# feifeibear/long-context-attention

Measured on AMD Instinct MI355X. Metric: attention TFLOP/s (algorithmic, causal fwd+bwd) + iter ms of LongContextAttention at seqlen 64K, ulysses x ring, higher is better.
Workload: dtype bf16

## Files before the change

long-context-attention_amd/csrc/usp_flash_fwd64.hip:

```cpp
#ifdef USP_F64_TIMING
#define USP_TIMING
#endif
#include "usp_fwd_params.hpp"
#include "usp_host.hpp"
#include "usp_mfma64.hpp"

namespace usp {

#ifndef USP_F64_NEA
#define USP_F64_NEA 42
#endif
constexpr int kF64_NEA = USP_F64_NEA;
#ifndef USP_F64_LEAD
#define USP_F64_LEAD 2
#endif
constexpr int kF64_LEAD = USP_F64_LEAD;
#ifndef USP_F64_PFK
#define USP_F64_PFK 2
#endif
constexpr int kF64_PFK = USP_F64_PFK;
#ifndef USP_F64_PFV
#define USP_F64_PFV 2
#endif
constexpr int kF64_PFV = USP_F64_PFV;
#ifndef USP_F64_MAX0
#define USP_F64_MAX0 22
#endif
constexpr int kF64_MAX0 = USP_F64_MAX0;
#ifndef USP_F64_DMA0
#define USP_F64_DMA0 2
#endif
constexpr int kF64_DMA0 = USP_F64_DMA0;
#ifndef USP_F64_DMAS
#define USP_F64_DMAS 6
#endif
constexpr int kF64_DMAS = USP_F64_DMAS;


template <int DT, bool CAUSAL, bool SPLIT = false>
__global__ __launch_bounds__(256, 1) void flash_fwd64_kernel(const FwdArgsT<SPLIT> ) {
  using E = Elem<DT>;
  using M = M64<DT>;
  constexpr int D = 128;
  constexpr int kBM = 256;
  constexpr int ROWB = D * 2;
  constexpr int KBYTES = kBN * ROWB;
  constexpr int NKT = D / 16;
  constexpr int NDJ = D / 32;
  constexpr int VOFF = 2 * KBYTES;

  extern __shared__ __attribute__((aligned(16))) char smem_raw[];
  USP_LDS char* smem = (USP_LDS char*)smem_raw;

  const int tid = threadIdx.x;
  const int lane = tid & 63;
  const int wave = __builtin_amdgcn_readfirstlane(tid >> 6);
  const int l31 = lane & 31;
  const int hi = lane >> 5;
  typedef const __attribute__((address_space(4))) FwdArgsT<SPLIT>* KArgs;
  KArgs p = (KArgs)__builtin_amdgcn_kernarg_segment_ptr();
  asm volatile("" : "+s"(p));

  const int k_voff = (16 * wave + (lane >> 4)) * (int)p->k_ss * 2 + (((lane & 15) ^ (lane >> 4)) * 16);
  const int v_voff = (16 * wave + ((lane & 15) >> 2)) * (int)p->v_ss * 2 + (32 * (lane >> 4) + 8 * (lane & 3)) * 2;
  const int k_rd = l31 * ROWB + ((hi ^ (l31 & 15)) * 16);
  const int v_rd = VOFF + hi * NDJ * 256 + ((lane & 15) >> 2) * 64 + ((lane >> 4) & 1) * 32 + (lane & 3) * 8;
  const float c = p->scale_log2;

  const ItemWalk walk(p->n_items);
  for (int pass = 0;; ++pass) {
  int w = walk.at(pass);
  if (w < 0) break;
  asm volatile("" : "+s"(p));
  int ks = 0;
  if constexpr (SPLIT) {
    w = walk.dealt(w, p->nq * p->ksplit);
    ks = w % p->ksplit; w /= p->ksplit;
  } else {
    w = walk.grouped(walk.dealt(w, p->nq), p->nq, p->walk_g);
  }
  const int qt_r = w % p->nq;
  int rest = w / p->nq;
  const int qt = CAUSAL ? (p->nq - 1 - qt_r) : qt_r;
  const int g = rest % p->G;
  rest /= p->G;
  const int hkv = rest % p->Hkv;
  const int b = rest / p->Hkv;
  const int h = hkv * p->G + g;

  const int q0 = qt * kBM;
  const int qw = q0 + wave * 64;
  int off = p->causal_off;
  int kb = 0, sk_cut = 0;
  if constexpr (SPLIT) {
    int e = p->Sk;
    if (CAUSAL) e = usp_rows_key_end(q0, kBM, p->Sq, e, 1, off);
    const int nt_all = usp_tiles_holding(e, kBN);
    kb = usp_prop_cut_tile(nt_all, p->ksplit, ks) * kBN;
    int ke = (ks == p->ksplit - 1) ? p->Sk : usp_prop_cut_tile(nt_all, p->ksplit, ks + 1) * kBN;
    ke = ke < p->Sk ? ke : p->Sk;
    sk_cut = ke > kb ? ke - kb : 0;
    off -= kb;
  }
  auto n_keys = [&]() { if constexpr (SPLIT) return sk_cut; else return p->Sk; };

  int blk_kv_end = n_keys(), wave_kv_end = n_keys();
  if (CAUSAL) {
    const int blk_last = (q0 + kBM < p->Sq ? q0 + kBM : p->Sq) - 1;
    const int wav_last = (qw + 64 < p->Sq ? qw + 64 : p->Sq) - 1;
    blk_kv_end = blk_last + off + 1 < n_keys() ? blk_last + off + 1 : n_keys();
    wave_kv_end = wav_last + off + 1 < n_keys() ? wav_last + off + 1 : n_keys();
  }
  if (qw >= p->Sq) wave_kv_end = 0;
  const int nt = usp_tiles_holding(blk_kv_end, kBN);
  int n_full = usp_unmasked_tiles(qw, n_keys(), CAUSAL, off, kBN);
  if (n_full > nt) n_full = nt;

USP_TM(
  const uint64_t tm_item = __builtin_amdgcn_s_memtime();
)
  u32x4 qf[2][NKT];
#pragma unroll
  for (int qb = 0; qb < 2; ++qb) {
    const int row = qw + 32 * qb + l31;
    const int row_c = row < p->Sq ? row : p->Sq - 1;
    const char* qp = p->q + 2 * (b * p->q_sb + (int64_t)row_c * p->q_ss + h * p->q_sh) + 16 * hi;
#pragma unroll
    for (int t = 0; t < NKT; ++t) qf[qb][t] = *(const u32x4*)(qp + 32 * t);
  }
#pragma unroll
  for (int qb = 0; qb < 2; ++qb)
#pragma unroll
    for (int t = 0; t < NKT; ++t) pin_agpr4(qf[qb][t]);

  const int64_t k_tb = (int64_t)kBN * p->k_ss * 2, v_tb = (int64_t)kBN * p->v_ss * 2;
  const char* k_cur = p->k + 2 * (b * p->k_sb + hkv * p->k_sh);
  const char* v_cur = p->v + 2 * (b * p->v_sb + hkv * p->v_sh);
  if constexpr (SPLIT) { k_cur += 2 * (int64_t)kb * p->k_ss; v_cur += 2 * (int64_t)kb * p->v_ss; }
  int rows_kv = n_keys();
  const int k_rowb = (int)p->k_ss * 2, v_rowb = (int)p->v_ss * 2;
  int lds_w = wave * 4096, k_step = 4 * (int)p->k_ss * 2 - 1024, v_step = 4 * (int)p->v_ss * 2 - 1024;
  u32x4 k_rs, v_rs;
  int k_ahead = 0;
  int dma_kbuf = 0, dma_vbuf = 0;
  auto dma_open = [&](int kbuf, int vbuf) {
    k_rs = make_rsrc_rows(k_cur, rows_kv + kBN * k_ahead, kBN, k_rowb, 2 * D);
    v_rs = make_rsrc_rows(v_cur, rows_kv, kBN, v_rowb, 2 * D);
    k_cur += k_tb;
    v_cur += v_tb;
    rows_kv -= kBN;
    dma_kbuf = kbuf; dma_vbuf = vbuf;
  };
  auto dma_open_k = [&](int kbuf) {
    k_rs = make_rsrc_rows(k_cur, rows_kv, kBN, k_rowb, 2 * D);
    k_cur += k_tb;
    k_ahead = -1;
    dma_kbuf = kbuf;
  };
  auto dma_piece = [&](int n) {
    asm volatile("" : "+s"(lds_w), "+s"(k_step), "+s"(v_step));
    if (n < 4) lds_dma16_asm(k_rs, lds_w + dma_kbuf * KBYTES, k_voff ^ (64 * n), n * k_step, n);
    else lds_dma16_asm(v_rs, lds_w + VOFF + dma_vbuf * KBYTES, v_voff, (n - 4) * v_step, n - 4);
  };
  auto dma_all = [&](int kbuf, int vbuf) {
    dma_open(kbuf, vbuf);
#pragma unroll
    for (int n = 0; n < 8; ++n) dma_piece(n);
  };

  f32x16 o[2][NDJ];
#pragma unroll
  for (int qb = 0; qb < 2; ++qb)
#pragma unroll
    for (int dj = 0; dj < NDJ; ++dj) zero_pin_agpr(o[qb][dj]);
  float m_run[2] = {USP_NEG_INF, USP_NEG_INF};
  float l_run[2] = {0.f, 0.f};

  auto qk = [&](int kbuf, f32x16 (&s)[2][2]) {
#pragma unroll
    for (int kt = 0; kt < NKT; ++kt) {
      USP_LDS const char* kp = smem + kbuf * KBYTES + (k_rd ^ (32 * kt));
      const u32x4 k0 = *(USP_LDS const u32x4*)kp;
      const u32x4 k1 = *(USP_LDS const u32x4*)(kp + 32 * ROWB);
#pragma unroll
      for (int qb = 0; qb < 2; ++qb) {
        if (kt == 0) { M::template s_first<true>(s[qb][0], k0, qf[qb][0]); M::template s_first<true>(s[qb][1], k1, qf[qb][0]); }
        else { M::template s_next<true>(s[qb][0], k0, qf[qb][kt]); M::template s_next<true>(s[qb][1], k1, qf[qb][kt]); }
      }
    }
    mfma_settle(s);
  };
  auto mask = [&](int kt0, f32x16 (&s)[2][2]) {
#pragma unroll
    for (int qb = 0; qb < 2; ++qb) {
      const int row = qw + 32 * qb + l31;
      int klim = n_keys() - 1;
      if (CAUSAL) klim = row + off < klim ? row + off : klim;
      const int kb0 = kt0 + 4 * hi;
#pragma unroll
      for (int r = 0; r < 16; ++r) {
        const int key = kb0 + (r & 3) + 8 * (r >> 2);
        if (key > klim) s[qb][0][r] = USP_NEG_INF;
        if (key + 32 > klim) s[qb][1][r] = USP_NEG_INF;
      }
    }
  };
  f32x16 sa[2][2], sb[2][2];
#pragma unroll
  for (int qb = 0; qb < 2; ++qb)
#pragma unroll
    for (int kb = 0; kb < 2; ++kb)
#pragma unroll
      for (int r = 0; r < 16; ++r) { sa[qb][kb][r] = 0.f; sb[qb][kb][r] = 0.f; }
  dma_all(0, 0);
  dma_open_k(1);
#pragma unroll
  for (int n = 0; n < 4; ++n) dma_piece(n);
  dma_drain();
  __syncthreads();
  if (nt > 0 && wave_kv_end > 0) qk(0, sa);
  __syncthreads();

  constexpr float kThr = 8.f;
  constexpr int NA = 32, NB = 32;
  constexpr int NEA = kF64_NEA, LEAD = kF64_LEAD, PFK = kF64_PFK, PFV = kF64_PFV, MAX0 = kF64_MAX0;
  constexpr int DMA0 = kF64_DMA0, DMAS = kF64_DMAS;
  static_assert(64 - NEA <= 22, "k-step 3 of P must be complete two slots before slot 24 of phase B");
  static_assert(MAX0 >= 1 && MAX0 < NB && DMAS >= 1 && DMA0 + 7 * DMAS < NA + NB, "");
  const float thr_raw = kThr / c;
  float m_thr[2] = {USP_NEG_INF, USP_NEG_INF};
  float nmc[2] = {0.f, 0.f};
  auto first_ref = [&](const float (&mt_lane)[2]) {
#pragma unroll
    for (int qb = 0; qb < 2; ++qb) {
      const float m_new = xhalf_max(mt_lane[qb]);
      const float m_use = (m_new == USP_NEG_INF) ? 0.f : m_new;
      m_run[qb] = m_new;
      m_thr[qb] = m_new + thr_raw;
      nmc[qb] = -(m_use * c);
    }
  };
  auto rescale = [&](const float (&mt_lane)[2]) {
    asm volatile("; rescale (rare)" ::: "memory");
    mfma_settle(o);
#pragma unroll
    for (int qb = 0; qb < 2; ++qb) {
      const float m_new = fmaxf(m_run[qb], xhalf_max(mt_lane[qb]));
      const float m_use = (m_new == USP_NEG_INF) ? 0.f : m_new;
      const float alpha = (m_new == m_run[qb]) ? 1.f : fast_exp2(m_run[qb] * c - m_use * c);
      m_run[qb] = m_new;
      m_thr[qb] = m_new + thr_raw;
      nmc[qb] = -(m_use * c);
      l_run[qb] *= alpha;
#pragma unroll
      for (int dj = 0; dj < NDJ; ++dj)
#pragma unroll
        for (int r = 0; r < 16; ++r) o[qb][dj][r] *= alpha;
    }
#pragma unroll
    for (int qb = 0; qb < 2; ++qb)
#pragma unroll
      for (int dj = 0; dj < NDJ; ++dj) pin_agpr(o[qb][dj]);
    operand_settle();
  };
  auto decide = [&](f32x16 (&s)[2][2]) {
    float mt[2];
#pragma unroll
    for (int qb = 0; qb < 2; ++qb) {
      mt[qb] = s[qb][0][0];
#pragma unroll
      for (int r = 1; r < 16; ++r) mt[qb] = fmaxf(mt[qb], s[qb][0][r]);
#pragma unroll
      for (int r = 0; r < 16; ++r) mt[qb] = fmaxf(mt[qb], s[qb][1][r]);
    }
    first_ref(mt);
  };
  auto iter = [&](auto par_c, auto mode_c, int jpar, int kt0_next, f32x16 (&cs)[2][2], f32x16 (&ns)[2][2])
      __attribute__((always_inline)) {
    constexpr int PARV = decltype(par_c)::value, MODE = decltype(mode_c)::value;
    const int par = PARV < 2 ? PARV : jpar;
    dma_open(par, par ^ 1);
    auto dma_slot = [&](int g) {
      if (g >= DMA0 && (g - DMA0) % DMAS == 0 && (g - DMA0) / DMAS < 8) dma_piece((g - DMA0) / DMAS);
    };
    USP_LDS const char* kb = smem + (par ^ 1) * KBYTES;
    USP_LDS const char* vb = smem + par * KBYTES + v_rd;
    int kr = k_rd;
    asm volatile("" : "+v"(kr));
    u32x4 ka[2 * NKT];
    auto rd_k = [&](int f) {
      ka[f] = *(USP_LDS const u32x4*)(kb + (f & 1) * 32 * ROWB + (kr ^ (32 * (f >> 1))));
    };
    u32x4 va[4 * NDJ];
    auto rd_v = [&](int f) {
      USP_LDS const char* vp = vb + (4 * (f / NDJ) * NDJ + (f % NDJ)) * 256;
      const u32x2 v0 = lds_read_tr16(vp);
      const u32x2 v1 = lds_read_tr16(vp + 2 * NDJ * 256);
      va[f] = u32x4{v0[0], v0[1], v1[0], v1[1]};
    };
    float rs[2] = {0.f, 0.f};
    u32x4 pf[2][4];
    auto get = [&](int e) -> float { return cs[(e >> 3) & 1][e >> 5][8 * ((e >> 4) & 1) + (e & 7)]; };
    auto consume = [&](int e) {
      rs[(e >> 3) & 1] += get(e);
      if (e & 1) pf[(e >> 3) & 1][e >> 4][(e & 7) >> 1] = E::pack2(get(e - 1), get(e));
    };
    auto exp_elem = [&](int e) {
      cs[(e >> 3) & 1][e >> 5][8 * ((e >> 4) & 1) + (e & 7)] = fast_exp2(__builtin_fmaf(get(e), c, nmc[(e >> 3) & 1]));
      if (e > 0) consume(e - 1);
      if (e == 63) consume(63);
    };
    if (MODE != 2) {
#pragma unroll
      for (int f = 0; f < PFK; ++f) rd_k(f);
    }
#pragma unroll
    for (int e = 0; e < LEAD; ++e) exp_elem(e);
    __builtin_amdgcn_sched_barrier(0);
#pragma unroll
    for (int sl = 0; sl < NA; ++sl) {
      const int f = sl >> 1, kt = f >> 1, kbk = f & 1, qb = sl & 1;
      if (MODE != 2) {
        if (qb == 0 && f + PFK < 2 * NKT) rd_k(f + PFK);
        if (kt == 0) M::template s_first<MODE != 0>(ns[qb][kbk], ka[f], qf[qb][0]);
        else M::template s_next<MODE != 0>(ns[qb][kbk], ka[f], qf[qb][kt]);
      }
#pragma unroll
      for (int e = LEAD + sl * (NEA - LEAD) / NA; e < LEAD + (sl + 1) * (NEA - LEAD) / NA; ++e) exp_elem(e);
      if (sl >= NA - 2 * PFV && ((sl - (NA - 2 * PFV)) & 1) == 0) rd_v((sl - (NA - 2 * PFV)) >> 1);
      dma_slot(sl);
      __builtin_amdgcn_sched_barrier(0);
    }
    if (MODE == 1) {
      mfma_settle(ns);
      mask(kt0_next, ns);
    }
    float mt[2] = {USP_NEG_INF, USP_NEG_INF};
    bool keep = true;
    constexpr int NMAX = NB - MAX0;
#pragma unroll
    for (int i = 0; i < NB; ++i) {
      const int f = i >> 1, qb = i & 1;
      if (qb == 0 && f + PFV < 4 * NDJ) rd_v(f + PFV);
      M::template o_acc<MODE != 0>(o[qb][f % NDJ], va[f], pf[qb][f / NDJ]);
      if (NEA + i < 64) exp_elem(NEA + i);
      if (i == 64 - NEA - 1 || (NEA == 64 && i == 0)) { l_run[0] += rs[0]; l_run[1] += rs[1]; }
      if (MODE != 2 && i >= MAX0) {
#pragma unroll
        for (int x = (i - MAX0) * 64 / NMAX; x < (i - MAX0 + 1) * 64 / NMAX; ++x)
          mt[x >> 5] = fmaxf(mt[x >> 5], ns[x >> 5][(x >> 4) & 1][x & 15]);
        if (i == NB - 1) keep = __all(mt[0] <= m_thr[0] && mt[1] <= m_thr[1]);
      }
      dma_slot(NA + i);
      __builtin_amdgcn_sched_barrier(0);
    }
    if (!keep) rescale(mt);
    dma_drain();
    __syncthreads();
  };

  const int n_w = usp_tiles_holding(wave_kv_end, kBN);
  if (n_full > n_w) n_full = n_w;
  int j = 0;
USP_TM(
  const uint64_t tm_loop = __builtin_amdgcn_s_memtime();
  uint64_t tm_hot = tm_loop;
)
  if (n_w > 0) {
    if (n_full == 0) mask(0, sa);
    decide(sa);
    const std::integral_constant<int, 0> c0;
    const std::integral_constant<int, 1> c1;
    const std::integral_constant<int, 2> c2;
    const int n_hot = n_full - 1;
    for (; j + 1 < n_hot; j += 2) {
      iter(c0, c0, 0, 0, sa, sb);
      iter(c1, c0, 1, 0, sb, sa);
    }
    auto adopt = [&]() {
#pragma unroll
      for (int qb = 0; qb < 2; ++qb)
#pragma unroll
        for (int kb = 0; kb < 2; ++kb) sa[qb][kb] = sb[qb][kb];
    };
USP_TM(
    tm_hot = __builtin_amdgcn_s_memtime();
)
    if (j < n_hot) { iter(c0, c0, 0, 0, sa, sb); adopt(); ++j; }
    for (; j < n_w; ++j) {
      if (j + 1 >= n_w) iter(c2, c2, j & 1, 0, sa, sb);
      else { iter(c2, c1, j & 1, (j + 1) * kBN, sa, sb); adopt(); }
    }
  }
USP_TM(
  const uint64_t tm_own = __builtin_amdgcn_s_memtime();
)
  for (; j < nt; ++j) {
    dma_all(j & 1, (j + 1) & 1);
    dma_drain();
    __syncthreads();
  }

USP_TM(
  const uint64_t tm_idle = __builtin_amdgcn_s_memtime();
)
  mfma_settle(o);
  asm volatile("" : "+s"(p));
#pragma unroll
  for (int qb = 0; qb < 2; ++qb) {
    const int row = qw + 32 * qb + l31;
    const float l_tot = xhalf_sum(l_run[qb]);
    const bool empty = !(l_tot > 0.f);
    const float inv = empty ? 0.f : 1.f / l_tot;
    const float blk_lse = empty ? USP_NEG_INF : (m_run[qb] * c + log2f(l_tot)) * kLn2;
    float w_blk = inv, w_old = 0.f, new_lse = blk_lse;
    float* lse_p = p->lse + b * p->lse_sb + h * p->lse_sh + row;
    if constexpr (SPLIT) lse_p += (int64_t)ks * p->B * p->Hq * p->Sq;
    const bool valid = row < p->Sq;
    const bool fin = row >= p->final_begin && row < p->final_end;
    const bool wide = !p->merge_in && p->out_wide && __all(!valid || fin);
    if (valid) {
      if (p->merge_in) {
        const float old = *lse_p;
        const float mx = fmaxf(old, blk_lse);
        if (mx == USP_NEG_INF) {
          new_lse = USP_NEG_INF; w_old = 0.f; w_blk = 0.f;
        } else {
          const float e_old = exp2f((old - mx) * kLog2e);
          const float e_blk = exp2f((blk_lse - mx) * kLog2e);
          const float sum = e_old + e_blk;
          new_lse = mx + log2f(sum) * kLn2;
          w_old = e_old / sum;
          w_blk = e_blk / sum * inv;
        }
      }
      if (hi == 0) *lse_p = new_lse;
      int64_t arow = b * p->a_sb + (int64_t)row * p->a_ss + h * p->a_sh;
      if constexpr (SPLIT) arow += (int64_t)ks * p->B * p->Sq * p->Hq * D;
      const int64_t orow = b * p->o_sb + (int64_t)row * p->o_ss + h * p->o_sh;
      if (wide) {
        char* op = p->out + 2 * orow;
#pragma unroll
        for (int dj = 0; dj < NDJ; ++dj)
#pragma unroll
          for (int g2 = 0; g2 < 2; ++g2) {
            const int r0 = 8 * g2;
            uint32_t ax = E::pack2(o[qb][dj][r0] * w_blk, o[qb][dj][r0 + 1] * w_blk);
            uint32_t ay = E::pack2(o[qb][dj][r0 + 2] * w_blk, o[qb][dj][r0 + 3] * w_blk);
            uint32_t bx = E::pack2(o[qb][dj][r0 + 4] * w_blk, o[qb][dj][r0 + 5] * w_blk);
            uint32_t by = E::pack2(o[qb][dj][r0 + 6] * w_blk, o[qb][dj][r0 + 7] * w_blk);
            const auto sx = __builtin_amdgcn_permlane32_swap(ax, bx, false, false);
            const auto sy = __builtin_amdgcn_permlane32_swap(ay, by, false, false);
            *(u32x4*)(op + 2 * (32 * dj + 16 * g2 + 8 * hi)) = u32x4{sx[0], sy[0], sx[1], sy[1]};
          }
      } else {
#pragma unroll
        for (int dj = 0; dj < NDJ; ++dj) {
#pragma unroll
          for (int g4 = 0; g4 < 4; ++g4) {
            const int d0 = 32 * dj + 8 * g4 + 4 * hi;
            f32x4 val = {o[qb][dj][4 * g4] * w_blk, o[qb][dj][4 * g4 + 1] * w_blk, o[qb][dj][4 * g4 + 2] * w_blk,
                         o[qb][dj][4 * g4 + 3] * w_blk};
            if (p->merge_in) {
              const f32x4 a = *(const f32x4*)(p->acc + arow + d0);
              val += a * w_old;
            }
            if (fin) {
              u32x2 pk = {E::pack2(val[0], val[1]), E::pack2(val[2], val[3])};
              *(u32x2*)(p->out + 2 * (orow + d0)) = pk;
            } else {
              *(f32x4*)(p->acc + arow + d0) = val;
            }
          }
        }
      }
    }
  }
USP_TM(
  {
    const uint64_t tm_end = __builtin_amdgcn_s_memtime();
    if (lane == 0 && (blockIdx.x % 61) == 0 && pass < 4)
      printf("TF wg %3d pass %d wave %d qt %2d tiles own %3d wg %3d : prologue %6llu hot-loop %8llu (%5llu / tile) tail-tiles %6llu idle %6llu epilogue %6llu\n",
             (int)blockIdx.x, pass, wave, qt, n_w, nt, (unsigned long long)(tm_loop - tm_item), (unsigned long long)(tm_hot - tm_loop),
             (unsigned long long)((tm_hot - tm_loop) / (n_full > 2 ? (n_full - 1) / 2 * 2 : 1)), (unsigned long long)(tm_own - tm_hot),
             (unsigned long long)(tm_idle - tm_own), (unsigned long long)(tm_end - tm_idle));
  }
)
  }
}

template <bool SPLIT>
static int launch64(FwdArgsT<SPLIT>& p, int dtype, bool causal, hipStream_t st) {
  p.nq = (p.Sq + 255) / 256;
  p.n_items = p.B * p.Hq * p.nq;
  if constexpr (SPLIT) p.n_items *= p.ksplit;
  const int grid = persistent_grid(p.n_items, device_cus(), p.interleave);
  const size_t lds = 2 * 2 * kBN * 128 * 2;
  with_dtype_causal(dtype, causal, [&](auto dt, auto c) {
    hipLaunchKernelGGL((flash_fwd64_kernel<decltype(dt)::value, decltype(c)::value, SPLIT>), dim3(grid), dim3(256), lds, st, p);
  });
  return launched();
}

bool launch_fwd64(const FwdArgsT<true>& p_in, int dtype, bool causal, hipStream_t st, int* rc) {
  if (!dma_rows_ok(p_in.k_ss, true) || !dma_rows_ok(p_in.v_ss, false)) return false;
  if (p_in.win_on || p_in.seq_q) return false;
  if (p_in.ksplit > 1) {
    FwdArgsT<true> p = p_in;
    p.acc = p.ws_o;
    p.a_sb = (int64_t)p.Sq * p.Hq * 128; p.a_ss = (int64_t)p.Hq * 128; p.a_sh = 128;
    p.lse = p.ws_lse;
    p.lse_sb = (int64_t)p.Hq * p.Sq; p.lse_sh = p.Sq;
    p.merge_in = 0; p.final_begin = 0; p.final_end = 0; p.out_wide = 0;
    *rc = launch64(p, dtype, causal, st);
    if (*rc == USP_OK) *rc = launch_split_merge(p_in, dtype, 128, st);
  } else {
    FwdArgsT<false> p;
    static_cast<FwdParams&>(p) = p_in;
    *rc = launch64(p, dtype, causal, st);
  }
  return true;
}

}
```

long-context-attention_amd/csrc/usp_mfma64.hpp:

```cpp
#pragma once
#include "usp_common.hpp"

#ifdef USP_TIMING
#define USP_TM(...) __VA_ARGS__
#else
#define USP_TM(...)
#endif

namespace usp {

USP_DEV USP_LDS char* lds_block_at_zero(char* smem_raw) {
  if ((uint32_t)(uintptr_t)(USP_LDS char*)smem_raw != 0u) __builtin_trap();
  return (USP_LDS char*)(uintptr_t)0;
}

template <int DT> struct M64;
#if defined(__HIP_DEVICE_COMPILE__)
#define USP_M64_BODY(MN)                                                                                              \
              \
   \
   \
  template <bool SAFE = false> static USP_DEV void s_first(f32x16& s, const u32x4& a, const u32x4& q) {               \
    if (SAFE) asm volatile("s_nop 1\n\t" MN " %0, %1, %2, 0" : "=&v"(s) : "v"(a), "a"(q));                          \
    else asm volatile(MN " %0, %1, %2, 0" : "=&v"(s) : "v"(a), "a"(q));                                               \
  }                                                                                                                   \
            \
  template <bool SAFE = false> static USP_DEV void s_first_c(f32x16& s, const u32x4& a, const u32x4& q, const f32x16& c) { \
    if (SAFE) asm volatile("s_nop 1\n\t" MN " %0, %1, %2, %3" : "=&v"(s) : "v"(a), "a"(q), "v"(c));                \
    else asm volatile(MN " %0, %1, %2, %3" : "=&v"(s) : "v"(a), "a"(q), "v"(c));                                      \
  }                                                                                                                   \
  template <bool SAFE = false> static USP_DEV void s_next(f32x16& s, const u32x4& a, const u32x4& q) {                \
    if (SAFE) asm volatile("s_nop 1\n\t" MN " %0, %1, %2, %0" : "+v"(s) : "v"(a), "a"(q));                          \
    else asm volatile(MN " %0, %1, %2, %0" : "+v"(s) : "v"(a), "a"(q));                                               \
  }                                                                                                                   \
                                             \
  template <bool SAFE = false> static USP_DEV void o_acc(f32x16& o, const u32x4& a, const u32x4& b) {                 \
    if (SAFE) asm volatile("s_nop 1\n\t" MN " %0, %1, %2, %0" : "+a"(o) : "v"(a), "v"(b));                          \
    else asm volatile(MN " %0, %1, %2, %0" : "+a"(o) : "v"(a), "v"(b));                                               \
  }
#else
#define USP_M64_BODY(MN)                                                                                              \
  template <bool SAFE = false> static USP_DEV void s_first(f32x16&, const u32x4&, const u32x4&) {}                    \
  template <bool SAFE = false> static USP_DEV void s_first_c(f32x16&, const u32x4&, const u32x4&, const f32x16&) {}   \
  template <bool SAFE = false> static USP_DEV void s_next(f32x16&, const u32x4&, const u32x4&) {}                     \
  template <bool SAFE = false> static USP_DEV void o_acc(f32x16&, const u32x4&, const u32x4&) {}
#endif
template <> struct M64<0> { USP_M64_BODY("v_mfma_f32_32x32x16_bf16") };
template <> struct M64<1> { USP_M64_BODY("v_mfma_f32_32x32x16_f16") };

USP_DEV void pin_agpr4(u32x4& x) {
#if defined(__HIP_DEVICE_COMPILE__)
  asm volatile("" : "+a"(x));
#endif
}
USP_DEV void zero_pin_agpr(f32x16& o) {
#pragma unroll
  for (int r = 0; r < 16; ++r) o[r] = 0.f;
  pin_agpr(o);
}
USP_DEV void load_resident16(u32x4 (&f0)[8], u32x4 (&f1)[8], const char* r0, const char* r1) {
#if defined(__HIP_DEVICE_COMPILE__)
  asm volatile("global_load_dwordx4 %0, %16, off\n\tglobal_load_dwordx4 %1, %16, off offset:32\n\t"
               "global_load_dwordx4 %2, %16, off offset:64\n\tglobal_load_dwordx4 %3, %16, off offset:96\n\t"
               "global_load_dwordx4 %4, %16, off offset:128\n\tglobal_load_dwordx4 %5, %16, off offset:160\n\t"
               "global_load_dwordx4 %6, %16, off offset:192\n\tglobal_load_dwordx4 %7, %16, off offset:224\n\t"
               "global_load_dwordx4 %8, %17, off\n\tglobal_load_dwordx4 %9, %17, off offset:32\n\t"
               "global_load_dwordx4 %10, %17, off offset:64\n\tglobal_load_dwordx4 %11, %17, off offset:96\n\t"
               "global_load_dwordx4 %12, %17, off offset:128\n\tglobal_load_dwordx4 %13, %17, off offset:160\n\t"
               "global_load_dwordx4 %14, %17, off offset:192\n\tglobal_load_dwordx4 %15, %17, off offset:224\n\t"
               "s_waitcnt vmcnt(0)"
               : "=&a"(f0[0]), "=&a"(f0[1]), "=&a"(f0[2]), "=&a"(f0[3]), "=&a"(f0[4]), "=&a"(f0[5]), "=&a"(f0[6]), "=&a"(f0[7]),
                 "=&a"(f1[0]), "=&a"(f1[1]), "=&a"(f1[2]), "=&a"(f1[3]), "=&a"(f1[4]), "=&a"(f1[5]), "=&a"(f1[6]), "=&a"(f1[7])
               : "v"(r0), "v"(r1) : "memory");
#endif
}
USP_DEV void mfma_settle(f32x16 (&o)[2][4]) {
#if defined(__HIP_DEVICE_COMPILE__)
  asm volatile("s_nop 15" : "+a"(o[0][0]), "+a"(o[0][1]), "+a"(o[0][2]), "+a"(o[0][3]),
                            "+a"(o[1][0]), "+a"(o[1][1]), "+a"(o[1][2]), "+a"(o[1][3]));
#endif
}
USP_DEV void mfma_settle(f32x16 (&s)[2][2]) {
  asm volatile("s_nop 15" : "+v"(s[0][0]), "+v"(s[0][1]), "+v"(s[1][0]), "+v"(s[1][1]));
}
USP_DEV void mfma_settle(f32x16 (&s)[2]) { asm volatile("s_nop 15" : "+v"(s[0]), "+v"(s[1])); }
USP_DEV void operand_settle() { asm volatile("s_nop 3" ::: "memory"); }

USP_DEV int dma_lane_col(int l15, int row) { return (l15 ^ (row << 2)) * 16; }
template <int D> USP_DEV int tile_swz(int row);
template <int D> USP_DEV int tr_read_offset(int i, int grp, int hi, int dj, int e) {
  const int rr = 8 * e + 4 * hi + (i >> 2);
  const int slot = 4 * dj + 2 * grp + ((i & 3) >> 1);
  return rr * (D * 2) + ((slot ^ tile_swz<D>(rr)) * 16) + (i & 1) * 8;
}

USP_DEV void lds_dma16_asm(const u32x4& rsrc, int lds_dst, int voffset, int soffset, int piece) {
#if defined(__HIP_DEVICE_COMPILE__)
  if (piece == 0)
    asm volatile("s_mov_b32 m0, %0\n\ts_nop 0\n\tbuffer_load_dwordx4 %1, %2, %3 offen lds"
                 : : "s"(lds_dst), "v"(voffset), "s"(rsrc), "s"(soffset) : "memory");
  if (piece == 1) asm volatile("buffer_load_dwordx4 %0, %1, %2 offen offset:1024 lds" : : "v"(voffset), "s"(rsrc), "s"(soffset) : "memory");
  if (piece == 2) asm volatile("buffer_load_dwordx4 %0, %1, %2 offen offset:2048 lds" : : "v"(voffset), "s"(rsrc), "s"(soffset) : "memory");
  if (piece == 3) asm volatile("buffer_load_dwordx4 %0, %1, %2 offen offset:3072 lds" : : "v"(voffset), "s"(rsrc), "s"(soffset) : "memory");
#endif
}
USP_DEV void lds_dma4_asm(const u32x4& rsrc, int lds_dst, int voffset) {
#if defined(__HIP_DEVICE_COMPILE__)
  asm volatile("s_mov_b32 m0, %0\n\ts_nop 0\n\tbuffer_load_dword %1, %2, 0 offen lds"
               : : "s"(lds_dst), "v"(voffset), "s"(rsrc) : "memory");
#endif
}
USP_DEV u32x4 make_rsrc(const char* base, int64_t bytes) {
  const uint64_t a = (uint64_t)base;
  const uint32_t n = bytes <= 0 ? 0u : (bytes > 0xffffffffLL ? 0xffffffffu : (uint32_t)bytes);
  return u32x4{(uint32_t)a, (uint32_t)(a >> 32) & 0xffffu, n, 0x00020000u};
}

USP_DEV u32x4 make_rsrc_rows(const char* base, int rows, int tile_rows, int row_bytes, int used) {
  const uint64_t a = (uint64_t)base;
  const int r = rows < tile_rows ? rows : tile_rows;
  const int n = r * row_bytes - (row_bytes - used);
  return u32x4{(uint32_t)a, (uint32_t)(a >> 32) & 0xffffu, (uint32_t)(n > 0 ? n : 0), 0x00020000u};
}

template <class E, int NDJ>
USP_DEV void store_row16_wide(char* row, const f32x16 (&t)[NDJ], float mul, int hi, bool valid) {
#if defined(__HIP_DEVICE_COMPILE__)
#pragma unroll
  for (int dj = 0; dj < NDJ; ++dj)
#pragma unroll
    for (int g2 = 0; g2 < 2; ++g2) {
      const int r0 = 8 * g2;
      const uint32_t ax = E::pack2(t[dj][r0] * mul, t[dj][r0 + 1] * mul);
      const uint32_t ay = E::pack2(t[dj][r0 + 2] * mul, t[dj][r0 + 3] * mul);
      const uint32_t bx = E::pack2(t[dj][r0 + 4] * mul, t[dj][r0 + 5] * mul);
      const uint32_t by = E::pack2(t[dj][r0 + 6] * mul, t[dj][r0 + 7] * mul);
      const auto sx = __builtin_amdgcn_permlane32_swap(ax, bx, false, false);
      const auto sy = __builtin_amdgcn_permlane32_swap(ay, by, false, false);
      if (valid) *(u32x4*)(row + 2 * (32 * dj + 16 * g2 + 8 * hi)) = u32x4{sx[0], sy[0], sx[1], sy[1]};
    }
#endif
}
template <class E, int NDJ>
USP_DEV void store_row32_acc(float* o32, char* o16, const f32x16 (&t)[NDJ], float mul, int hi, int accf) {
#pragma unroll
  for (int dj = 0; dj < NDJ; ++dj)
#pragma unroll
    for (int g4 = 0; g4 < 4; ++g4) {
      const int d0 = 32 * dj + 8 * g4 + 4 * hi;
      f32x4 v = {t[dj][4 * g4] * mul, t[dj][4 * g4 + 1] * mul, t[dj][4 * g4 + 2] * mul, t[dj][4 * g4 + 3] * mul};
      if (accf) v += *(const f32x4*)(o32 + d0);
      if (o16) *(u32x2*)(o16 + 2 * d0) = u32x2{E::pack2(v[0], v[1]), E::pack2(v[2], v[3])};
      else *(f32x4*)(o32 + d0) = v;
    }
}

}
```

Baseline: 1011.

## Stage K/V fragments in a fixed AGPR bank for plain flash-forward iterations

For the unmasked (MODE 0) hot-loop iterations, K and V fragments are loaded from LDS directly into a fixed bank of accumulation registers (a192-a255) with inline asm. The MFMAs then read that bank in batches of eight fragments, each batch guarded by one lgkmcnt(0) wait, instead of the earlier rolling two-fragment prefetch into compiler-managed VGPRs. The goal is to deepen LDS prefetch and cut per-fragment wait and dependency stalls without adding VGPR pressure. The cost is hand-pinned register allocation, coarser waits, and reliance on constant LDS offsets (lds_block_at_zero). Timing probes are also added under the timing macro.

New measurement: 1019 (median of 6 runs). About the same (+0.8%).

```diff
diff --git a/long-context-attention_amd/csrc/usp_flash_fwd64.hip b/long-context-attention_amd/csrc/usp_flash_fwd64.hip
--- a/long-context-attention_amd/csrc/usp_flash_fwd64.hip
+++ b/long-context-attention_amd/csrc/usp_flash_fwd64.hip
@@ -15,14 +15,6 @@
 #define USP_F64_LEAD 2
 #endif
 constexpr int kF64_LEAD = USP_F64_LEAD;
-#ifndef USP_F64_PFK
-#define USP_F64_PFK 2
-#endif
-constexpr int kF64_PFK = USP_F64_PFK;
-#ifndef USP_F64_PFV
-#define USP_F64_PFV 2
-#endif
-constexpr int kF64_PFV = USP_F64_PFV;
 #ifndef USP_F64_MAX0
 #define USP_F64_MAX0 22
 #endif
@@ -36,11 +28,20 @@
 #endif
 constexpr int kF64_DMAS = USP_F64_DMAS;
 
+#ifdef USP_TIMING
+USP_DEV uint32_t tm_stamp() {
+  __builtin_amdgcn_sched_barrier(0);
+  const uint32_t t = (uint32_t)__builtin_amdgcn_s_memtime();
+  __builtin_amdgcn_sched_barrier(0);
+  return t;
+}
+#endif
 
 template <int DT, bool CAUSAL, bool SPLIT = false>
 __global__ __launch_bounds__(256, 1) void flash_fwd64_kernel(const FwdArgsT<SPLIT> ) {
   using E = Elem<DT>;
   using M = M64<DT>;
+  using MB = M64Bank<DT>;
   constexpr int D = 128;
   constexpr int kBM = 256;
   constexpr int ROWB = D * 2;
@@ -50,7 +51,7 @@
   constexpr int VOFF = 2 * KBYTES;
 
   extern __shared__ __attribute__((aligned(16))) char smem_raw[];
-  USP_LDS char* smem = (USP_LDS char*)smem_raw;
+  USP_LDS char* smem = lds_block_at_zero(smem_raw);
 
   const int tid = threadIdx.x;
   const int lane = tid & 63;
@@ -221,9 +222,11 @@
   if (nt > 0 && wave_kv_end > 0) qk(0, sa);
   __syncthreads();
 
+  USP_TM(uint32_t tm_grp[7] = {0, 0, 0, 0, 0, 0, 0};)
   constexpr float kThr = 8.f;
   constexpr int NA = 32, NB = 32;
-  constexpr int NEA = kF64_NEA, LEAD = kF64_LEAD, PFK = kF64_PFK, PFV = kF64_PFV, MAX0 = kF64_MAX0;
+  constexpr int NEA = kF64_NEA, LEAD = kF64_LEAD, MAX0 = kF64_MAX0;
+  constexpr int PFK = 2, PFV = 2;
   constexpr int DMA0 = kF64_DMA0, DMAS = kF64_DMAS;
   static_assert(64 - NEA <= 22, "k-step 3 of P must be complete two slots before slot 24 of phase B");
   static_assert(MAX0 >= 1 && MAX0 < NB && DMAS >= 1 && DMA0 + 7 * DMAS < NA + NB, "");
@@ -279,24 +282,33 @@
       __attribute__((always_inline)) {
     constexpr int PARV = decltype(par_c)::value, MODE = decltype(mode_c)::value;
     const int par = PARV < 2 ? PARV : jpar;
+    USP_TM(uint32_t tm_s[7] = {0, 0, 0, 0, 0, 0, 0}; if (MODE == 0) tm_s[0] = tm_stamp();)
     dma_open(par, par ^ 1);
     auto dma_slot = [&](int g) {
       if (g >= DMA0 && (g - DMA0) % DMAS == 0 && (g - DMA0) / DMAS < 8) dma_piece((g - DMA0) / DMAS);
     };
+    constexpr bool BANK = MODE == 0;
+    static_assert(!BANK || PARV < 2, "the plain iterations know their parity");
     USP_LDS const char* kb = smem + (par ^ 1) * KBYTES;
     USP_LDS const char* vb = smem + par * KBYTES + v_rd;
     int kr = k_rd;
     asm volatile("" : "+v"(kr));
     u32x4 ka[2 * NKT];
-    auto rd_k = [&](int f) {
-      ka[f] = *(USP_LDS const u32x4*)(kb + (f & 1) * 32 * ROWB + (kr ^ (32 * (f >> 1))));
+    auto rd_k = [&](int f) __attribute__((always_inline)) {
+      if (BANK) frag_read_b128(frag_reg((f >> 3) & 1, f & 7), kr ^ (32 * (f >> 1)), ((PARV ^ 1) & 1) * KBYTES + (f & 1) * 32 * ROWB);
+      else ka[f] = *(USP_LDS const u32x4*)(kb + (f & 1) * 32 * ROWB + (kr ^ (32 * (f >> 1))));
     };
     u32x4 va[4 * NDJ];
-    auto rd_v = [&](int f) {
-      USP_LDS const char* vp = vb + (4 * (f / NDJ) * NDJ + (f % NDJ)) * 256;
-      const u32x2 v0 = lds_read_tr16(vp);
-      const u32x2 v1 = lds_read_tr16(vp + 2 * NDJ * 256);
-      va[f] = u32x4{v0[0], v0[1], v1[0], v1[1]};
+    auto rd_v = [&](int f) __attribute__((always_inline)) {
+      if (BANK) {
+        const int o0 = (PARV & 1) * KBYTES + (4 * (f / NDJ) * NDJ + (f % NDJ)) * 256;
+        frag_read_tr16x2(frag_reg((f >> 3) & 1, f & 7), v_rd, o0, o0 + 2 * NDJ * 256);
+      } else {
+        USP_LDS const char* vp = vb + (4 * (f / NDJ) * NDJ + (f % NDJ)) * 256;
+        const u32x2 v0 = lds_read_tr16(vp);
+        const u32x2 v1 = lds_read_tr16(vp + 2 * NDJ * 256);
+        va[f] = u32x4{v0[0], v0[1], v1[0], v1[1]};
+      }
     };
     float rs[2] = {0.f, 0.f};
     u32x4 pf[2][4];
@@ -312,7 +324,7 @@
     };
     if (MODE != 2) {
 #pragma unroll
-      for (int f = 0; f < PFK; ++f) rd_k(f);
+      for (int f = 0; f < (BANK ? 8 : PFK); ++f) rd_k(f);
     }
 #pragma unroll
     for (int e = 0; e < LEAD; ++e) exp_elem(e);
@@ -320,14 +332,22 @@
 #pragma unroll
     for (int sl = 0; sl < NA; ++sl) {
       const int f = sl >> 1, kt = f >> 1, kbk = f & 1, qb = sl & 1;
-      if (MODE != 2) {
+      if (BANK) {
+        USP_TM(if (sl == 16) tm_s[2] = tm_stamp();)
+        if ((sl & 15) == 0) frag_wait();
+        USP_TM(if (sl == 0) tm_s[1] = tm_stamp();)
+        if (kt == 0) MB::template s_first<false>(ns[qb][kbk], frag_reg(f >> 3, f & 7), qf[qb][0]);
+        else MB::template s_next<false>(ns[qb][kbk], frag_reg(f >> 3, f & 7), qf[qb][kt]);
+        if (sl < 4) { rd_k(8 + 2 * sl); rd_k(9 + 2 * sl); }
+        if (sl >= 16 && sl < 24) rd_v(sl - 16);
+      } else if (MODE != 2) {
         if (qb == 0 && f + PFK < 2 * NKT) rd_k(f + PFK);
-        if (kt == 0) M::template s_first<MODE != 0>(ns[qb][kbk], ka[f], qf[qb][0]);
-        else M::template s_next<MODE != 0>(ns[qb][kbk], ka[f], qf[qb][kt]);
+        if (kt == 0) M::template s_first<true>(ns[qb][kbk], ka[f], qf[qb][0]);
+        else M::template s_next<true>(ns[qb][kbk], ka[f], qf[qb][kt]);
       }
 #pragma unroll
       for (int e = LEAD + sl * (NEA - LEAD) / NA; e < LEAD + (sl + 1) * (NEA - LEAD) / NA; ++e) exp_elem(e);
-      if (sl >= NA - 2 * PFV && ((sl - (NA - 2 * PFV)) & 1) == 0) rd_v((sl - (NA - 2 * PFV)) >> 1);
+      if (!BANK && sl >= NA - 2 * PFV && ((sl - (NA - 2 * PFV)) & 1) == 0) rd_v((sl - (NA - 2 * PFV)) >> 1);
       dma_slot(sl);
       __builtin_amdgcn_sched_barrier(0);
     }
@@ -341,8 +361,15 @@
 #pragma unroll
     for (int i = 0; i < NB; ++i) {
       const int f = i >> 1, qb = i & 1;
-      if (qb == 0 && f + PFV < 4 * NDJ) rd_v(f + PFV);
-      M::template o_acc<MODE != 0>(o[qb][f % NDJ], va[f], pf[qb][f / NDJ]);
+      if (BANK) {
+        USP_TM(if ((i & 15) == 0) tm_s[3 + i / 16] = tm_stamp();)
+        if ((i & 15) == 0) frag_wait();
+        MB::template o_acc<false>(o[qb][f % NDJ], frag_reg(f >> 3, f & 7), pf[qb][f / NDJ]);
+        if (i < 8) rd_v(8 + i);
+      } else {
+        if (qb == 0 && f + PFV < 4 * NDJ) rd_v(f + PFV);
+        M::template o_acc<true>(o[qb][f % NDJ], va[f], pf[qb][f / NDJ]);
+      }
       if (NEA + i < 64) exp_elem(NEA + i);
       if (i == 64 - NEA - 1 || (NEA == 64 && i == 0)) { l_run[0] += rs[0]; l_run[1] += rs[1]; }
       if (MODE != 2 && i >= MAX0) {
@@ -354,9 +381,15 @@
       dma_slot(NA + i);
       __builtin_amdgcn_sched_barrier(0);
     }
+    USP_TM(if (MODE == 0) tm_s[5] = tm_stamp();)
     if (!keep) rescale(mt);
     dma_drain();
     __syncthreads();
+    USP_TM(if (MODE == 0) {
+      tm_s[6] = tm_stamp();
+      _Pragma("unroll") for (int x = 0; x < 6; ++x) tm_grp[x] += tm_s[x + 1] - tm_s[x];
+      ++tm_grp[6];
+    })
   };
 
   const int n_w = usp_tiles_holding(wave_kv_end, kBN);
@@ -480,10 +513,13 @@
   {
     const uint64_t tm_end = __builtin_amdgcn_s_memtime();
     if (lane == 0 && (blockIdx.x % 61) == 0 && pass < 4)
-      printf("TF wg %3d pass %d wave %d qt %2d tiles own %3d wg %3d : prologue %6llu hot-loop %8llu (%5llu / tile) tail-tiles %6llu idle %6llu epilogue %6llu\n",
+      printf("TF wg %3d pass %d wave %d qt %2d tiles own %3d wg %3d : prologue %6llu hot-loop %8llu (%5llu / tile) tail-tiles %6llu idle %6llu epilogue %6llu"
+             " | plain tiles %u: lead %u A0 %u A1 %u B0 %u B1 %u drain+barrier %u\n",
              (int)blockIdx.x, pass, wave, qt, n_w, nt, (unsigned long long)(tm_loop - tm_item), (unsigned long long)(tm_hot - tm_loop),
              (unsigned long long)((tm_hot - tm_loop) / (n_full > 2 ? (n_full - 1) / 2 * 2 : 1)), (unsigned long long)(tm_own - tm_hot),
-             (unsigned long long)(tm_idle - tm_own), (unsigned long long)(tm_end - tm_idle));
+             (unsigned long long)(tm_idle - tm_own), (unsigned long long)(tm_end - tm_idle), tm_grp[6],
+             tm_grp[0] / (tm_grp[6] ? tm_grp[6] : 1), tm_grp[1] / (tm_grp[6] ? tm_grp[6] : 1), tm_grp[2] / (tm_grp[6] ? tm_grp[6] : 1),
+             tm_grp[3] / (tm_grp[6] ? tm_grp[6] : 1), tm_grp[4] / (tm_grp[6] ? tm_grp[6] : 1), tm_grp[5] / (tm_grp[6] ? tm_grp[6] : 1));
   }
 )
   }
diff --git a/long-context-attention_amd/csrc/usp_mfma64.hpp b/long-context-attention_amd/csrc/usp_mfma64.hpp
--- a/long-context-attention_amd/csrc/usp_mfma64.hpp
+++ b/long-context-attention_amd/csrc/usp_mfma64.hpp
@@ -47,6 +47,50 @@
 #endif
 template <> struct M64<0> { USP_M64_BODY("v_mfma_f32_32x32x16_bf16") };
 template <> struct M64<1> { USP_M64_BODY("v_mfma_f32_32x32x16_f16") };
+
+#define USP_FRAG_BANK_CLOBBER                                                                                          \
+  "a192", "a193", "a194", "a195", "a196", "a197", "a198", "a199", "a200", "a201", "a202", "a203", "a204", "a205", "a206", "a207", \
+  "a208", "a209", "a210", "a211", "a212", "a213", "a214", "a215", "a216", "a217", "a218", "a219", "a220", "a221", "a222", "a223", \
+  "a224", "a225", "a226", "a227", "a228", "a229", "a230", "a231", "a232", "a233", "a234", "a235", "a236", "a237", "a238", "a239", \
+  "a240", "a241", "a242", "a243", "a244", "a245", "a246", "a247", "a248", "a249", "a250", "a251", "a252", "a253", "a254", "a255"
+constexpr int kFragBank0 = 192;
+constexpr int frag_reg(int bank, int slot) { return kFragBank0 + 32 * bank + 4 * slot; }
+#if defined(__HIP_DEVICE_COMPILE__)
+USP_DEV void frag_read_b128(int r, int addr, int off) {
+  asm volatile("ds_read_b128 a[%c1:%c2], %0 offset:%c3" : : "v"(addr), "i"(r), "i"(r + 3), "i"(off) : "memory");
+}
+USP_DEV void frag_read_tr16x2(int r, int addr, int off0, int off1) {
+  asm volatile("ds_read_b64_tr_b16 a[%c1:%c2], %0 offset:%c5\n\tds_read_b64_tr_b16 a[%c3:%c4], %0 offset:%c6"
+               : : "v"(addr), "i"(r), "i"(r + 1), "i"(r + 2), "i"(r + 3), "i"(off0), "i"(off1) : "memory");
+}
+USP_DEV void frag_wait() { asm volatile("s_waitcnt lgkmcnt(0)" : : : "memory", USP_FRAG_BANK_CLOBBER); }
+template <int DT> struct M64Bank;
+#define USP_M64_BANK_BODY(MN)                                                                                         \
+                                                       \
+  template <bool SAFE = false> static USP_DEV void s_first(f32x16& s, int r, const u32x4& q) {                        \
+    if (SAFE) asm volatile("s_nop 1\n\t" MN " %0, a[%c2:%c3], %1, 0" : "=&v"(s) : "a"(q), "i"(r), "i"(r + 3));      \
+    else asm volatile(MN " %0, a[%c2:%c3], %1, 0" : "=&v"(s) : "a"(q), "i"(r), "i"(r + 3));                           \
+  }                                                                                                                   \
+  template <bool SAFE = false> static USP_DEV void s_next(f32x16& s, int r, const u32x4& q) {                         \
+    if (SAFE) asm volatile("s_nop 1\n\t" MN " %0, a[%c2:%c3], %1, %0" : "+v"(s) : "a"(q), "i"(r), "i"(r + 3));      \
+    else asm volatile(MN " %0, a[%c2:%c3], %1, %0" : "+v"(s) : "a"(q), "i"(r), "i"(r + 3));                           \
+  }                                                                                                                   \
+  template <bool SAFE = false> static USP_DEV void o_acc(f32x16& o, int r, const u32x4& b) {                          \
+    if (SAFE) asm volatile("s_nop 1\n\t" MN " %0, a[%c2:%c3], %1, %0" : "+a"(o) : "v"(b), "i"(r), "i"(r + 3));      \
+    else asm volatile(MN " %0, a[%c2:%c3], %1, %0" : "+a"(o) : "v"(b), "i"(r), "i"(r + 3));                           \
+  }
+template <> struct M64Bank<0> { USP_M64_BANK_BODY("v_mfma_f32_32x32x16_bf16") };
+template <> struct M64Bank<1> { USP_M64_BANK_BODY("v_mfma_f32_32x32x16_f16") };
+#else
+USP_DEV void frag_read_b128(int, int, int) {}
+USP_DEV void frag_read_tr16x2(int, int, int, int) {}
+USP_DEV void frag_wait() {}
+template <int DT> struct M64Bank {
+  template <bool SAFE = false> static USP_DEV void s_first(f32x16&, int, const u32x4&) {}
+  template <bool SAFE = false> static USP_DEV void s_next(f32x16&, int, const u32x4&) {}
+  template <bool SAFE = false> static USP_DEV void o_acc(f32x16&, int, const u32x4&) {}
+};
+#endif
 
 USP_DEV void pin_agpr4(u32x4& x) {
 #if defined(__HIP_DEVICE_COMPILE__)
```
